# CEA-LIST/runia_core

Hardware: AMD Instinct MI355X
Metric: OOD scores/sec, LaREM 16-MC PCA-256 (ResNet-18 layer4 latent 512x4x4) (higher is better)
Workload: dtype f64

## Files before the change

### runia_core_amd/csrc/entropy_core.hpp

```cpp
#pragma once
#include "common.hpp"

namespace runia_entropy {

constexpr double kInf = __builtin_inf();

inline double digamma_diff(int n, int k) {
  double s = 0.0;
  for (int j = n - 1; j >= k; --j) s += 1.0 / (double)j;
  return s;
}

__device__ __forceinline__ void cswap(float& a, float& b) {
  float lo, hi;
  asm("v_min_f32 %0, %1, %2" : "=v"(lo) : "v"(a), "v"(b));
  asm("v_max_f32 %0, %1, %2" : "=v"(hi) : "v"(a), "v"(b));
  a = lo;
  b = hi;
}
__device__ __forceinline__ void cswap(double& a, double& b) {
  double lo, hi;
  asm("v_min_f64 %0, %1, %2" : "=v"(lo) : "v"(a), "v"(b));
  asm("v_max_f64 %0, %1, %2" : "=v"(hi) : "v"(a), "v"(b));
  a = lo;
  b = hi;
}

__device__ __forceinline__ void sort3(float& a, float& b, float& c) {
  float lo, md, hi;
  asm("v_min3_f32 %0, %1, %2, %3" : "=v"(lo) : "v"(a), "v"(b), "v"(c));
  asm("v_med3_f32 %0, %1, %2, %3" : "=v"(md) : "v"(a), "v"(b), "v"(c));
  asm("v_max3_f32 %0, %1, %2, %3" : "=v"(hi) : "v"(a), "v"(b), "v"(c));
  a = lo;
  b = md;
  c = hi;
}
__device__ __forceinline__ void sort3(double& a, double& b, double& c) {
  cswap(a, b);
  cswap(b, c);
  cswap(a, b);
}

template <int OFF, int NP, typename T>
__device__ __forceinline__ void sort16_at(T (&v)[NP]) {
#define RUNIA_S3(a, b, c) sort3(v[OFF + a], v[OFF + b], v[OFF + c]);
  RUNIA_S3(6, 7, 15) RUNIA_S3(10, 12, 13) RUNIA_S3(0, 2, 3) RUNIA_S3(1, 4, 5) RUNIA_S3(9, 11, 14)
  RUNIA_S3(3, 5, 15) RUNIA_S3(8, 13, 14) RUNIA_S3(2, 4, 7) RUNIA_S3(8, 10, 11) RUNIA_S3(9, 10, 12)
  RUNIA_S3(5, 7, 14) RUNIA_S3(0, 1, 6) RUNIA_S3(11, 12, 13) RUNIA_S3(3, 4, 6) RUNIA_S3(1, 2, 3)
  RUNIA_S3(5, 6, 13) RUNIA_S3(0, 8, 9) RUNIA_S3(1, 8, 9) RUNIA_S3(3, 7, 11) RUNIA_S3(13, 14, 15)
  RUNIA_S3(11, 12, 13) RUNIA_S3(4, 8, 11) RUNIA_S3(5, 7, 9) RUNIA_S3(2, 6, 10) RUNIA_S3(6, 7, 8)
  RUNIA_S3(3, 5, 6) RUNIA_S3(2, 3, 4) RUNIA_S3(9, 10, 11)
#undef RUNIA_S3
}

template <int OFF, int NP, typename T>
__device__ __forceinline__ void merge16x2_at(T (&v)[NP]) {
#define RUNIA_S3(a, b, c) sort3(v[OFF + a], v[OFF + b], v[OFF + c]);
#define RUNIA_S2(a, b) cswap(v[OFF + a], v[OFF + b]);
  RUNIA_S2(10, 26) RUNIA_S3(14, 26, 30) RUNIA_S3(12, 26, 28) RUNIA_S3(4, 12, 20) RUNIA_S3(0, 4, 16)
  RUNIA_S3(1, 4, 17) RUNIA_S3(3, 17, 19) RUNIA_S3(2, 10, 18) RUNIA_S3(15, 30, 31) RUNIA_S3(6, 10, 22)
  RUNIA_S3(5, 17, 21) RUNIA_S3(2, 3, 4) RUNIA_S3(13, 21, 29) RUNIA_S3(7, 19, 23) RUNIA_S3(11, 19, 27)
  RUNIA_S3(9, 21, 25) RUNIA_S3(7, 9, 17) RUNIA_S3(8, 20, 24) RUNIA_S3(15, 23, 27) RUNIA_S3(6, 7, 16)
  RUNIA_S3(11, 13, 17) RUNIA_S3(14, 18, 22) RUNIA_S3(8, 12, 16) RUNIA_S3(15, 19, 21) RUNIA_S3(9, 10, 12)
  RUNIA_S2(5, 6) RUNIA_S3(21, 22, 24) RUNIA_S3(18, 19, 20) RUNIA_S3(23, 25, 26) RUNIA_S3(15, 17, 18)
  RUNIA_S3(27, 28, 29) RUNIA_S3(14, 15, 16) RUNIA_S2(23, 24) RUNIA_S2(13, 14) RUNIA_S2(11, 12)
#undef RUNIA_S2
#undef RUNIA_S3
}

template <int NP, typename T>
__device__ __forceinline__ void sort_asc(T (&v)[NP]) {
  static_assert((NP & (NP - 1)) == 0, "power of two");
  if constexpr (NP == 8) {
#define RUNIA_S3(a, b, c) sort3(v[a], v[b], v[c]);
    RUNIA_S3(0, 5, 6) RUNIA_S3(1, 2, 3) RUNIA_S3(4, 6, 7) RUNIA_S3(0, 1, 4) RUNIA_S3(2, 5, 6) RUNIA_S3(3, 6, 7) RUNIA_S3(3, 4, 5) RUNIA_S3(1, 2, 3)
#undef RUNIA_S3
  } else {
    if constexpr (NP >= 16) {
      sort16_at<0>(v);
      if constexpr (NP >= 32) sort16_at<16>(v);
      if constexpr (NP >= 64) { sort16_at<32>(v); sort16_at<48>(v); }
      static_assert(NP <= 64, "add the 16-blocks of a larger sort here");
    }
    if constexpr (NP >= 32) {
      merge16x2_at<0>(v);
      if constexpr (NP >= 64) merge16x2_at<32>(v);
    }
#pragma unroll
    for (int p = (NP >= 32 ? 32 : (NP >= 16 ? 16 : 1)); p < NP; p <<= 1) {
#pragma unroll
      for (int k = p; k >= 1; k >>= 1) {
#pragma unroll
        for (int j = k % p; j + k < NP; j += 2 * k) {
#pragma unroll
          for (int i = 0; i < k; ++i) {
            if (i + j + k < NP && (i + j) / (2 * p) == (i + j + k) / (2 * p)) cswap(v[i + j], v[i + j + k]);
          }
        }
      }
    }
  }
}

__device__ __forceinline__ double fma_scalar_addend(double a, double b, double c) {
  double r;
  asm("v_fma_f64 %0, %1, %2, %3" : "=v"(r) : "v"(a), "v"(b), "s"(c));
  return r;
}

__device__ __forceinline__ double log_mantissa(double x, int& e_out) {
  int e;
  double f = frexp(x, &e);
  const bool low = f < 0.70710678118654752440;
  f = low ? f + f : f;
  e_out = low ? e - 1 : e;
  const double num = f - 1.0, den = f + 1.0;
  double r = __builtin_amdgcn_rcp(den);
  r = fma(fma(-den, r, 1.0), r, r);
  r = fma(fma(-den, r, 1.0), r, r);
  double q = num * r;
  q = fma(fma(-den, q, num), r, q);
  const double t = q * q;
  double p = 1.0 / 21.0;
  p = fma_scalar_addend(p, t, 1.0 / 19.0);
  p = fma_scalar_addend(p, t, 1.0 / 17.0);
  p = fma_scalar_addend(p, t, 1.0 / 15.0);
  p = fma_scalar_addend(p, t, 1.0 / 13.0);
  p = fma_scalar_addend(p, t, 1.0 / 11.0);
  p = fma_scalar_addend(p, t, 1.0 / 9.0);
  p = fma_scalar_addend(p, t, 1.0 / 7.0);
  p = fma_scalar_addend(p, t, 1.0 / 5.0);
  p = fma_scalar_addend(p, t, 1.0 / 3.0);
  const double q2 = q + q;
  return fma(q2 * t, p, q2);
}

template <int NP, int K, bool FULL = false>
__device__ __forceinline__ double column_log_sum(const float (&vs)[NP], int n, double min_dist) {
  double v[NP];
#pragma unroll
  for (int i = 0; i < NP; ++i) v[i] = (double)vs[i];
  double gap[NP][K];
#pragma unroll
  for (int a = 0; a < NP; ++a)
#pragma unroll
    for (int m = 1; m <= K; ++m) gap[a][m - 1] = (a + m < NP) ? v[a + m] - v[a] : kInf;
  double mant = 1.0;
  int esum = 0;
#pragma unroll
  for (int i0 = 0; i0 < NP; i0 += 4) {
    double prod = 1.0;
#pragma unroll
    for (int i = i0; i < i0 + 4 && i < NP; ++i) {
      double e = kInf;
      bool first = true;
#pragma unroll
      for (int j = 0; j <= K; ++j) {
        const int li = i - j, ri = i + (K - j);
        if (li < 0 || ri >= NP) continue;
        double cand;
        if (j == 0) cand = gap[i][K - 1];
        else if (j == K) cand = gap[li][K - 1];
        else cand = fmax(gap[li][j - 1], gap[i][K - j - 1]);
        e = first ? cand : fmin(e, cand);
        first = false;
      }
      e = fmax(e, min_dist);
      if (FULL || i < n) prod *= e;
    }
    int ex;
    const double m = frexp(prod, &ex);
    mant *= m;
    esum += ex;
  }
  int em;
  const double lf = log_mantissa(mant, em);
  return fma((double)(esum + em + (FULL ? NP : n)), 0.69314718055994530942, lf);
}

}
```

### runia_core_amd/csrc/mc_sampler.hip

```cpp
#include <type_traits>

#include "common.hpp"
#include "entropy_core.hpp"
#include "philox.hpp"
#include "div_consts.hpp"
#include "roi_source.hpp"

namespace {

using namespace runia_entropy;

constexpr int kMaxMC = 64;
typedef float f2 __attribute__((ext_vector_type(2)));
typedef float f4 __attribute__((ext_vector_type(4)));

#ifndef K0_NT_STORE
#define K0_NT_STORE 0
#endif
#ifndef K1_NT_STORE
#define K1_NT_STORE 0
#endif
template <int NT, typename T>
__device__ __forceinline__ void store_out(T* p, T v) {
  if constexpr (NT != 0) __builtin_nontemporal_store(v, p);
  else *p = v;
}

__device__ __forceinline__ void layer_consts(int cnt, int& m, float& flag, float& zh, float& zl) {
  const int a = cnt ? __ffs(cnt) - 1 : 0;
  m = cnt >> a;
  flag = __uint_as_float((unsigned)(127 - a) << 23);
  zh = cnt ? __uint_as_float(runia_div::kDivHi[(m - 1) >> 1]) : NAN;
  zl = cnt ? __uint_as_float(runia_div::kDivLo[(m - 1) >> 1]) : 0.f;
}

__device__ __forceinline__ float add_f32(float a, float b) {
  float r;
  asm("v_add_f32 %0, %1, %2" : "=v"(r) : "v"(a), "v"(b));
  return r;
}

__device__ __forceinline__ float div_newton(float u, float den, float r) {
  const float q = u * r;
  const float e = fmaf(-den, q, u);
  return fmaf(e, r, q);
}

template <int HT, int WT>
__host__ __device__ constexpr int mask_slot(int p) {
  if constexpr (HT % 2 == 0) {
    const int y = p / WT, xw = p - y * WT;
    return ((y >> 1) * WT + xw) * 2 + (y & 1);
  } else {
    return p;
  }
}

template <int HT, int WT>
__host__ __device__ constexpr int slot_position(int slot) {
  if constexpr (HT % 2 == 0) {
    const int e = slot & 1, t = slot >> 1;
    const int k = t / WT, xw = t - k * WT;
    return (2 * k + e) * WT + xw;
  } else {
    return slot;
  }
}

template <int HT, int WT>
__device__ __forceinline__ unsigned long long columns_below(int k) {
  unsigned long long row = (k >= 64) ? ~0ull : ((1ull << k) - 1ull), m = 0ull;
#pragma unroll
  for (int y = 0; y < HT; ++y) m |= row << (y * WT);
  return m;
}

constexpr int kMaskBitsWaves = 4;

template <int HT, int WT, int NP, bool REDRAW = false>
__global__ __launch_bounds__(64 * kMaskBitsWaves) void mc_mask_bits_kernel(const float* __restrict__ rnd,
                                                                           int64_t rand_stride,
                                                                           float* __restrict__ table, int64_t N,
                                                                           int n_mc, float gamma, int block_size,
                                                                           int identity, int sort_layers,
                                                                           uint64_t rng_seed, int64_t first_image) {
  constexpr int HW = HT * WT;
  static_assert(HW <= 64 && NP <= 64, "one drop layer per 64-bit word");
  constexpr bool DIV = (64 % HW == 0);
  constexpr int WORDS = (NP * HW + 63) / 64;
  constexpr unsigned long long FULL = (HW == 64) ? ~0ull : ((1ull << HW) - 1ull);
  const int lane = threadIdx.x & 63;
  const int64_t img = (int64_t)blockIdx.x * kMaskBitsWaves + (threadIdx.x >> 6);
  if (img >= N) return;
  const int bit0 = lane * HW, word0 = bit0 >> 6, off = bit0 & 63;
  const int pad = block_size / 2;

  auto seeds_of = [&](unsigned attempt) -> unsigned long long {
    float d[WORDS];
    if (rnd) {
      const float* r = rnd + img * rand_stride;
#pragma unroll
      for (int t = 0; t < WORDS; ++t) {
        const int i = lane + 64 * t;
        d[t] = (i < n_mc * HW) ? r[i] : 1.0f;
      }
    } else {
#pragma unroll
      for (int q = 0; q < (WORDS + 3) / 4; ++q) {
        const runia_philox::u4 b = runia_philox::lane_block(rng_seed, (uint64_t)(first_image + img), lane, q, attempt);
#pragma unroll
        for (int j = 0; j < 4; ++j) {
          const int t = 4 * q + j;
          if (t < WORDS) d[t] = (lane + 64 * t < n_mc * HW) ? runia_philox::component(b, j) : 1.0f;
        }
      }
    }
    unsigned long long lo = 0ull, hi = 0ull;
#pragma unroll
    for (int t = 0; t < WORDS; ++t) {
      const unsigned long long w = __ballot(d[t] < gamma);
      if (t == word0) lo = w;
      if (!DIV && t == word0 + 1) hi = w;
    }
    unsigned long long sd = lo >> off;
    if (!DIV && off + HW > 64) sd |= hi << (64 - off);
    return sd & FULL;
  };
  auto keep_of = [&](unsigned long long seed) -> unsigned long long {
    unsigned long long hx = 0ull;
    for (int dx = 0; dx < block_size; ++dx) {
      const int ox = dx - pad;
      if (ox >= WT || -ox >= WT) continue;
      hx |= (ox >= 0) ? ((seed >> ox) & columns_below<HT, WT>(WT - ox))
                      : ((seed << -ox) & ~columns_below<HT, WT>(-ox) & FULL);
    }
    unsigned long long dropped = 0ull;
    for (int dy = 0; dy < block_size; ++dy) {
      const int oy = dy - pad;
      if (oy >= HT || -oy >= HT) continue;
      dropped |= (oy >= 0) ? (hx >> (oy * WT)) : ((hx << (-oy * WT)) & FULL);
    }
    return ~dropped & FULL;
  };

  unsigned long long keep = identity ? FULL : keep_of(seeds_of(0u));
  if (REDRAW && !identity && !rnd) {
    for (unsigned attempt = 1; attempt <= 16u; ++attempt) {
      if (__ballot(lane < n_mc && keep == 0ull) == 0ull) break;
      const unsigned long long again = keep_of(seeds_of(attempt));
      if (keep == 0ull) keep = again;
    }
  }
  const int cnt = __popcll(keep);
  int m;
  float flag, zh, zl;
  layer_consts(cnt, m, flag, zh, zl);
  const int key = m ? m : 127;
  int rank = 0;
#pragma unroll
  for (int j = 0; j < NP; ++j) {
    const int o = __shfl(key, j, 64);
    rank += (j < n_mc) && ((o < key) || (o == key && j < lane));
  }
  if (!sort_layers) rank = lane;
  if (lane >= n_mc) return;
  float* out = table + img * (int64_t)(n_mc * (HW + 2));
  float* rec = out + rank * HW;
  if constexpr (HW % 4 == 0) {
#pragma unroll
    for (int c = 0; c < HW / 4; ++c) {
      f4 v;
      v.x = ((keep >> slot_position<HT, WT>(4 * c)) & 1ull) ? flag : 0.f;
      v.y = ((keep >> slot_position<HT, WT>(4 * c + 1)) & 1ull) ? flag : 0.f;
      v.z = ((keep >> slot_position<HT, WT>(4 * c + 2)) & 1ull) ? flag : 0.f;
      v.w = ((keep >> slot_position<HT, WT>(4 * c + 3)) & 1ull) ? flag : 0.f;
      store_out<K0_NT_STORE>(reinterpret_cast<f4*>(rec) + c, v);
    }
  } else {
#pragma unroll
    for (int q = 0; q < HW; ++q)
      store_out<K0_NT_STORE>(rec + q, ((keep >> slot_position<HT, WT>(q)) & 1ull) ? flag : 0.f);
  }
  store_out<K0_NT_STORE>(out + n_mc * HW + rank, zh);
  store_out<K0_NT_STORE>(out + n_mc * (HW + 1) + rank, zl);
}

constexpr int kLutRecDwords = 20, kLutSortDword = 18, kLutOddDword = 19;
constexpr int kLutLayerShift = 23, kLutClassShift = 27;
constexpr unsigned kLutOffsetMask = (1u << kLutLayerShift) - 1u;
constexpr size_t kLutKeys = 65536;
static_assert((kLutKeys - 1) * kLutRecDwords * 4 <= kLutOffsetMask, "a record's byte offset fits below the layer index");
constexpr size_t kLutRecords = (kLutOffsetMask + 1) / (kLutRecDwords * 4) + 2;
static_assert(kLutRecords * kLutRecDwords * 4 >= kLutOffsetMask + 1 + kLutRecDwords * 4, "every masked offset reads inside the table");

void flag_lut_fill_4x4(uint32_t* out, int block_size) {
  constexpr int HT = 4, WT = 4, HW = 16;
  const int pad = block_size / 2;
  for (size_t i = kLutKeys * kLutRecDwords; i < kLutRecords * kLutRecDwords; ++i) out[i] = 0u;
  for (unsigned key = 0; key < kLutKeys; ++key) {
    unsigned keep = 0;
    for (int y = 0; y < HT; ++y)
      for (int xw = 0; xw < WT; ++xw) {
        bool dropped = false;
        for (int yy = 0; yy < HT; ++yy)
          for (int xx = 0; xx < WT; ++xx)
            if (((key >> (yy * WT + xx)) & 1u) && yy - y >= -pad && yy - y < block_size - pad && xx - xw >= -pad &&
                xx - xw < block_size - pad)
              dropped = true;
        if (!dropped) keep |= 1u << (y * WT + xw);
      }
    const int cnt = __builtin_popcount(keep);
    const int a = cnt ? __builtin_ctz((unsigned)cnt) : 0;
    const int m = cnt >> a;
    const uint32_t flag = (uint32_t)(127 - a) << 23;
    uint32_t* rec = out + (size_t)key * kLutRecDwords;
    for (int slot = 0; slot < HW; ++slot) rec[slot] = ((keep >> slot_position<HT, WT>(slot)) & 1u) ? flag : 0u;
    rec[HW] = cnt ? runia_div::kDivHiC[(m - 1) >> 1] : 0x7fc00000u;
    rec[HW + 1] = cnt ? runia_div::kDivLoC[(m - 1) >> 1] : 0u;
    const unsigned cls = cnt ? (unsigned)(m - 1) >> 1 : 8u;
    rec[kLutSortDword] = (cls << kLutClassShift) | (key * (unsigned)(kLutRecDwords * 4));
    rec[kLutOddDword] = (uint32_t)m;
  }
}

__device__ __forceinline__ void sort16_uniform(unsigned (&v)[16]) {
#pragma unroll
  for (int p = 1; p < 16; p <<= 1) {
#pragma unroll
    for (int k = p; k >= 1; k >>= 1) {
#pragma unroll
      for (int j = k % p; j + k < 16; j += 2 * k) {
#pragma unroll
        for (int i = 0; i < k; ++i) {
          if (i + j + k < 16 && (i + j) / (2 * p) == (i + j + k) / (2 * p)) {
            const unsigned lo = v[i + j] < v[i + j + k] ? v[i + j] : v[i + j + k];
            const unsigned hi = v[i + j] < v[i + j + k] ? v[i + j + k] : v[i + j];
            v[i + j] = lo;
            v[i + j + k] = hi;
          }
        }
      }
    }
  }
}

#ifndef K1_BLOCK
#define K1_BLOCK 128
#endif
constexpr int kK1Block = K1_BLOCK;


template <int HT, int WT, int G>
__device__ __forceinline__ void roi_load_map(float (&u)[HT * WT], const RoiSource* __restrict__ src, int64_t roi, int c) {
  typedef const __attribute__((address_space(4))) unsigned* cptr;
  cptr tab = (cptr)(src->table + roi * (int64_t)src->roi_dwords);
  const unsigned image = tab[0];
  const __amdgpu_buffer_rsrc_t rsrc = __builtin_amdgcn_make_buffer_rsrc(
      const_cast<float*>(src->nhwc) + (int64_t)image * (src->image_bytes / 4), 0, (int)src->image_bytes, 0x00020000);
  const int voff = c * 4;
  cptr rows = tab + 8, cols = tab + 8 + 4 * (HT * G);
  constexpr float count = (float)(G * G);
  constexpr int SX = WT * G, SY = HT * G;
  unsigned ox_lo[SX], ox_hi[SX];
  float hx[SX], lx[SX];
#pragma unroll
  for (int sx = 0; sx < SX; ++sx) {
    ox_lo[sx] = cols[4 * sx];
    ox_hi[sx] = cols[4 * sx + 1];
    hx[sx] = __uint_as_float(cols[4 * sx + 2]);
    lx[sx] = __uint_as_float(cols[4 * sx + 3]);
  }
  float acc[HT * WT];
#pragma unroll
  for (int p = 0; p < HT * WT; ++p) acc[p] = 0.f;
  float tl[SX][2], th[SX][2];
  unsigned cur_lo = 0xffffffffu, cur_hi = 0xffffffffu;
#pragma unroll
  for (int sy = 0; sy < SY; ++sy) {
    const unsigned oy_lo = rows[4 * sy], oy_hi = rows[4 * sy + 1];
    const float hy = __uint_as_float(rows[4 * sy + 2]), ly = __uint_as_float(rows[4 * sy + 3]);
    if (oy_lo != cur_lo || oy_hi != cur_hi) {
      if (oy_lo == cur_hi) {
#pragma unroll
        for (int sx = 0; sx < SX; ++sx) { tl[sx][0] = th[sx][0]; tl[sx][1] = th[sx][1]; }
      } else {
#pragma unroll
        for (int sx = 0; sx < SX; ++sx) {
          tl[sx][0] = __builtin_bit_cast(float, __builtin_amdgcn_raw_buffer_load_b32(rsrc, voff, (int)(oy_lo + ox_lo[sx]), 0));
          tl[sx][1] = __builtin_bit_cast(float, __builtin_amdgcn_raw_buffer_load_b32(rsrc, voff, (int)(oy_lo + ox_hi[sx]), 0));
        }
      }
#pragma unroll
      for (int sx = 0; sx < SX; ++sx) {
        th[sx][0] = __builtin_bit_cast(float, __builtin_amdgcn_raw_buffer_load_b32(rsrc, voff, (int)(oy_hi + ox_lo[sx]), 0));
        th[sx][1] = __builtin_bit_cast(float, __builtin_amdgcn_raw_buffer_load_b32(rsrc, voff, (int)(oy_hi + ox_hi[sx]), 0));
      }
      cur_lo = oy_lo;
      cur_hi = oy_hi;
    }
    __builtin_amdgcn_sched_barrier(0);
#pragma unroll
    for (int sx = 0; sx < SX; ++sx) {
      const float w1 = hy * hx[sx], w2 = hy * lx[sx], w3 = ly * hx[sx], w4 = ly * lx[sx];
      const float val = w1 * tl[sx][0] + w2 * tl[sx][1] + w3 * th[sx][0] + w4 * th[sx][1];
      float& bin = acc[(sy / G) * WT + (sx / G)];
      bin += val;
      asm volatile("" : "+v"(bin));
    }
  }
#pragma unroll
  for (int p = 0; p < HT * WT; ++p) u[p] = acc[p] / count;
}

#ifndef K1_IMGS
#define K1_IMGS 1
#endif
template <int HT, int WT, int NP, int K, bool FULL, bool ENTROPY, int ROI_G, bool ZOUT, bool LUT = false>
__device__ __forceinline__ void mc_entropy_item(const float* __restrict__ x, const float* __restrict__ table,
                                                double* __restrict__ h, float* __restrict__ z_out,
                                                double* __restrict__ zero_fill, int64_t N, int C, int n_mc_rt,
                                                double min_dist, double const_term, double inv_n, int64_t img, int c,
                                                const float* __restrict__ rnd = nullptr, int64_t rand_stride = 0,
                                                float gamma = 0.f) {
  constexpr int HW = HT * WT;
  constexpr bool PAIRS = (HT % 2 == 0);
  const int n_mc = FULL ? NP : n_mc_rt;
  if (img >= N) return;
  unsigned long long seedw[LUT ? NP * HW / 64 : 1];
  if constexpr (LUT) {
    static_assert(!LUT || (HW == 16 && NP == 16 && FULL && !ZOUT && ROI_G == 0), "the geometry table is for 4x4 x 16 layers");
    const float* r = rnd + img * rand_stride + (threadIdx.x & 63);
#pragma unroll
    for (int t = 0; t < NP * HW / 64; ++t) seedw[t] = __ballot(r[64 * t] < gamma);
  }
  if (zero_fill && c == 0) zero_fill[img] = 0.0;
  if (c >= C) return;
  typedef const __attribute__((address_space(4))) unsigned* lut_ptr;
  const lut_ptr lut = (lut_ptr) reinterpret_cast<const unsigned*>(table);
  unsigned sv[LUT ? NP : 1];
  if constexpr (LUT) {
#pragma unroll
    for (int s = 0; s < NP; ++s) {
      const unsigned key = (unsigned)(seedw[s >> 2] >> (16 * (s & 3))) & 0xffffu;
      sv[s] = lut[key * kLutRecDwords + kLutSortDword] | ((unsigned)s << kLutLayerShift);
    }
    sort16_uniform(sv);
  }
  const float* mk = table + img * (int64_t)(n_mc * (HW + 2));
  const float* zhs = mk + n_mc * HW;
  const float* zls = zhs + n_mc;
  float u[HW];
  if constexpr (ROI_G > 0) {
    roi_load_map<HT, WT, ROI_G>(u, reinterpret_cast<const RoiSource*>(x), img, c);
  } else {
    const float* xc = x + (img * C + c) * (int64_t)HW;
    if constexpr (HW % 4 == 0) {
#pragma unroll
      for (int p = 0; p < HW / 4; ++p) {
        const float4 v = reinterpret_cast<const float4*>(xc)[p];
        u[4 * p] = v.x; u[4 * p + 1] = v.y; u[4 * p + 2] = v.z; u[4 * p + 3] = v.w;
      }
    } else {
#pragma unroll
      for (int p = 0; p < HW; ++p) u[p] = xc[p];
    }
  }
  constexpr bool w_pow2 = (WT & (WT - 1)) == 0, h_pow2 = (HT & (HT - 1)) == 0;
  constexpr bool hw_pow2 = w_pow2 && h_pow2;
  if constexpr (!hw_pow2) {
#pragma unroll
    for (int p = 0; p < HW; ++p) u[p] *= (float)HW;
  }
  const float rW = 1.0f / (float)WT, rH = 1.0f / (float)HT;
  float z[NP];
  float q[PAIRS ? 1 : HW];
  f2 q2[PAIRS ? HW / 2 : 1];
  unsigned cur_zh_bits = __float_as_uint(1.0f);
#pragma unroll
  for (int p = 0; p < HW; ++p) {
    if constexpr (PAIRS) q2[mask_slot<HT, WT>(p) >> 1][mask_slot<HT, WT>(p) & 1] = u[p];
    else q[p] = u[p];
  }
#ifndef K1_GCAP
#define K1_GCAP 128
#endif
  constexpr int GCAP = FULL ? K1_GCAP : K1_GCAP / 2;
  constexpr int G = (GCAP / HW < 1) ? 1 : ((GCAP / HW > NP) ? NP : GCAP / HW);
  if constexpr (!(FULL && NP % G == 0)) {
#pragma unroll
    for (int s = 0; s < NP; ++s) z[s] = INFINITY;
  }
#ifndef K1_TRIP_UNROLL
#define K1_TRIP_UNROLL 1
#endif
#pragma unroll K1_TRIP_UNROLL
  for (int s0 = 0; s0 < NP; s0 += G) {
    float znew[G];
    float dg[G], rg[G], mg[G][HW];
    const float* mk_t = mk + (FULL ? s0 * HW : 0);
    const float* zhs_t = zhs + (FULL ? s0 : 0);
    const float* zls_t = zls + (FULL ? s0 : 0);
#pragma unroll
    for (int g = 0; g < G; ++g) {
      if constexpr (LUT) {
        const lut_ptr rec = lut + (sv[g] & kLutOffsetMask) / 4u;
        dg[g] = __uint_as_float(rec[HW]);
        rg[g] = __uint_as_float(rec[HW + 1]);
#pragma unroll
        for (int p = 0; p < HW; ++p) mg[g][p] = __uint_as_float(rec[p]);
      } else {
        const int sc = FULL ? g : ((s0 + g < n_mc) ? s0 + g : n_mc - 1);
        dg[g] = zhs_t[sc];
        rg[g] = zls_t[sc];
#pragma unroll
        for (int p = 0; p < HW; ++p) mg[g][p] = mk_t[sc * HW + p];
      }
    }
#pragma unroll
    for (int g = 0; g < G; ++g) {
      const int s = s0 + g;
      znew[g] = INFINITY;
      if (FULL || s < n_mc) {
        const float zh = dg[g], zl = rg[g];
        if (__float_as_uint(zh) != cur_zh_bits) {
#pragma unroll
          for (int p = 0; p < HW; ++p) {
            const float qv = fmaf(u[p], zh, u[p] * zl);
            if constexpr (PAIRS) q2[mask_slot<HT, WT>(p) >> 1][mask_slot<HT, WT>(p) & 1] = qv;
            else q[p] = qv;
          }
          cur_zh_bits = __float_as_uint(zh);
        }
        const float* m = mg[g];
        float col;
        if constexpr (PAIRS) {
          float rows[HT];
#pragma unroll
          for (int k2 = 0; k2 < HT / 2; ++k2) {
            const f2* qq = q2 + k2 * WT;
            const float* mm = m + 2 * k2 * WT;
            f2 acc = qq[0] * (f2){mm[0], mm[1]};
#pragma unroll
            for (int xi = 1; xi < WT; ++xi) {
              const int xw = torch_chain<WT>(xi);
              acc = __builtin_elementwise_fma(qq[xw], (f2){mm[2 * xw], mm[2 * xw + 1]}, acc);
            }
            if constexpr (hw_pow2) {
            } else if constexpr (w_pow2) {
              acc = acc * (f2){rW, rW};
            } else {
              acc = (f2){div_newton(acc.x, (float)WT, rW), div_newton(acc.y, (float)WT, rW)};
            }
            rows[2 * k2] = acc.x;
            rows[2 * k2 + 1] = acc.y;
          }
          col = rows[0];
#pragma unroll
          for (int yi = 1; yi < HT; ++yi) col = add_f32(col, rows[torch_chain<HT>(yi)]);
        } else {
          float rm[HT];
#pragma unroll
          for (int y = 0; y < HT; ++y) {
            float rowsum = q[y * WT] * m[y * WT];
#pragma unroll
            for (int xi = 1; xi < WT; ++xi) {
              const int xw = torch_chain<WT>(xi);
              rowsum = fmaf(q[y * WT + xw], m[y * WT + xw], rowsum);
            }
            rm[y] = w_pow2 ? rowsum * rW : div_newton(rowsum, (float)WT, rW);
          }
          col = rm[0];
#pragma unroll
          for (int yi = 1; yi < HT; ++yi) col += rm[torch_chain<HT>(yi)];
        }
        if constexpr (hw_pow2 && PAIRS) znew[g] = col;
        else znew[g] = h_pow2 ? col * rH : div_newton(col, (float)HT, rH);
        if constexpr (ZOUT) {
          if (z_out) z_out[(img * n_mc + s) * (int64_t)C + c] = znew[g];
        }
      }
    }
#pragma unroll
    for (int i = NP - 1; i >= G; --i) z[i] = z[i - G];
#pragma unroll
    for (int g = 0; g < G; ++g) z[g] = znew[g];
    if constexpr (LUT) {
#pragma unroll
      for (int g = 0; g + G < NP; ++g) sv[g] = sv[g + G];
    }
  }
  if constexpr (ENTROPY) {
    float nan_probe = z[0];
#pragma unroll
    for (int s = 1; s < NP; ++s) nan_probe += z[s];
    const bool bad = nan_probe != nan_probe;
    sort_asc<NP>(z);
    double res = const_term + inv_n * column_log_sum<NP, K, FULL>(z, n_mc, min_dist);
    if (bad) res = NAN;
    store_out<K1_NT_STORE>(h + (img * C + c), res);
  }
}

template <int HT, int WT, int NP, int K, bool FULL, bool ENTROPY, int ROI_G, bool ZOUT>
#ifdef K1_WAVES
__attribute__((amdgpu_waves_per_eu(K1_WAVES, 8)))
#endif
__global__ __launch_bounds__(kK1Block) void mc_entropy_kernel(const float* __restrict__ x,
                                                          const float* __restrict__ table,
                                                          double* __restrict__ h, float* __restrict__ z_out,
                                                          double* __restrict__ zero_fill, int64_t N, int C,
                                                          int n_mc_rt, double min_dist, double const_term,
                                                          double inv_n) {
  const unsigned chunks = (unsigned)(C + kK1Block - 1) / kK1Block;
  const unsigned slot = blockIdx.x >> 3;
  const int c = (int)(slot % chunks) * kK1Block + threadIdx.x;
#pragma unroll 1
  for (int rep = 0; rep < K1_IMGS; ++rep) {
    const int64_t img = ((int64_t)(slot / chunks) * K1_IMGS + rep) * 8 + (blockIdx.x & 7);
    mc_entropy_item<HT, WT, NP, K, FULL, ENTROPY, ROI_G, ZOUT>(x, table, h, z_out, zero_fill, N, C, n_mc_rt, min_dist,
                                                              const_term, inv_n, img, c);
  }
}

template <int HT, int WT, int NP, int K>
__attribute__((amdgpu_waves_per_eu(6, 8)))
__global__ __launch_bounds__(kK1Block) void mc_entropy_lut_kernel(const float* __restrict__ x,
                                                              const float* __restrict__ rnd, int64_t rand_stride,
                                                              const float* __restrict__ lut, float gamma,
                                                              double* __restrict__ h, double* __restrict__ zero_fill,
                                                              int64_t N, int C, double min_dist, double const_term,
                                                              double inv_n) {
  const unsigned chunks = (unsigned)(C + kK1Block - 1) / kK1Block;
  const unsigned slot = blockIdx.x >> 3;
  const int c = (int)(slot % chunks) * kK1Block + threadIdx.x;
#pragma unroll 1
  for (int rep = 0; rep < K1_IMGS; ++rep) {
    const int64_t img = ((int64_t)(slot / chunks) * K1_IMGS + rep) * 8 + (blockIdx.x & 7);
    mc_entropy_item<HT, WT, NP, K, true, true, 0, false, true>(x, lut, h, nullptr, zero_fill, N, C, NP, min_dist, const_term,
                                                               inv_n, img, c, rnd, rand_stride, gamma);
  }
}

template <int HT, int WT, int NP, int K, bool FULL, int ROI_G>
void launch_mc_entropy(unsigned grid, hipStream_t s, const float* x, const float* table, double* h, float* z_out,
                       double* zero_fill, int64_t N, int C, int n_mc, double min_dist, double ct, double inv_n) {
  auto go = [&](auto kernel) {
    if constexpr (ROI_G == 0)
      RUNIA_LAUNCH_TIMED(kernel, grid, kK1Block, 0, s, x, table, h, z_out, zero_fill, N, C, n_mc, min_dist, ct, inv_n);
    else
      hipLaunchKernelGGL(kernel, dim3(grid), dim3(kK1Block), 0, s, x, table, h, z_out, zero_fill, N, C, n_mc, min_dist, ct,
                         inv_n);
  };
  if constexpr (HT == 4 && WT == 4) {
    if (!z_out) return go(mc_entropy_kernel<HT, WT, NP, K, FULL, true, ROI_G, false>);
  }
  go(mc_entropy_kernel<HT, WT, NP, K, FULL, true, ROI_G, true>);
}

template <int HH, int WW, int NPP>
void launch_mask(const float* rnd, int64_t rand_image_stride, float* table, int64_t N, int n_mc, float gamma,
                 int block_size, int identity, int sort_layers, uint64_t seed, int64_t first_image, int redraw,
                 hipStream_t s) {
  static_assert(HH * WW <= 64, "mc_mask_bits_kernel holds a drop layer in one 64-bit word");
  const unsigned grid = (unsigned)((N + kMaskBitsWaves - 1) / kMaskBitsWaves);
  if (redraw)
    mc_mask_bits_kernel<HH, WW, NPP, true><<<grid, 64 * kMaskBitsWaves, 0, s>>>(rnd, rand_image_stride, table, N, n_mc, gamma,
                                                                              block_size, identity, sort_layers, seed, first_image);
  else
    mc_mask_bits_kernel<HH, WW, NPP, false><<<grid, 64 * kMaskBitsWaves, 0, s>>>(rnd, rand_image_stride, table, N, n_mc, gamma,
                                                                               block_size, identity, sort_layers, seed, first_image);
}

__global__ void mc_draws_kernel(float* __restrict__ out, int64_t N, int per_image, uint64_t seed, int64_t first_image) {
  const int64_t i = (int64_t)blockIdx.x * blockDim.x + threadIdx.x;
  if (i >= N * per_image) return;
  const int64_t img = i / per_image;
  out[i] = runia_philox::draw(seed, (uint64_t)(first_image + img), (int)(i - img * per_image));
}
}

extern "C" size_t runia_mc_entropy_workspace_bytes(int64_t N, int H, int W, int n_mc) {
  if (N <= 0 || H <= 0 || W <= 0 || n_mc <= 0) return 0;
  return (size_t)N * (size_t)n_mc * (size_t)(H * W + 2) * sizeof(float);
}

static unsigned k1_grid(int64_t N, int C) {
  return (unsigned)((((N + 7) / 8 + K1_IMGS - 1) / K1_IMGS) * 8 * ((C + kK1Block - 1) / kK1Block));
}

#define RUNIA_MCE_SHAPES(F) \
  F(4, 4, 16, 5) F(4, 4, 32, 5) F(4, 4, 8, 5) F(2, 2, 16, 5) F(2, 2, 32, 5) F(7, 7, 16, 5) F(7, 7, 32, 5) F(8, 8, 16, 5) F(8, 8, 32, 5)

#define RUNIA_ROI_MCE_SHAPES(X)                                                                                    \
  X(7, 7, 16, 5, 2) X(7, 7, 32, 5, 2) X(7, 7, 16, 5, 1) X(7, 7, 32, 5, 1)                                          \
  X(4, 4, 16, 5, 2) X(4, 4, 32, 5, 2) X(8, 8, 16, 5, 2) X(8, 8, 32, 5, 2)

template <int V> using int_c = std::integral_constant<int, V>;

template <class F>
int mc_for_shape(int H, int W, int n_mc, int k, F&& f, bool any_k = false) {
#define RUNIA_MCE(HH, WW, NPP, KK)                                                                 \
  if (H == HH && W == WW && n_mc <= NPP && n_mc > NPP / 2 && (k == KK || any_k)) {                \
    if (n_mc == NPP) f(int_c<HH>{}, int_c<WW>{}, int_c<NPP>{}, int_c<KK>{}, std::true_type{});     \
    else f(int_c<HH>{}, int_c<WW>{}, int_c<NPP>{}, int_c<KK>{}, std::false_type{});                \
    return 1;                                                                                      \
  }
  RUNIA_MCE_SHAPES(RUNIA_MCE)
#undef RUNIA_MCE
  return 0;
}

template <class F>
int roi_mc_for_shape(int PH, int PW, int n_mc, int k, int sampling_ratio, F&& f) {
#define RUNIA_ROI_MCE(HH, WW, NPP, KK, GG)                                                                    \
  if (PH == HH && PW == WW && n_mc <= NPP && n_mc > NPP / 2 && k == KK && sampling_ratio == GG) {             \
    if (n_mc == NPP) f(int_c<HH>{}, int_c<WW>{}, int_c<NPP>{}, int_c<KK>{}, int_c<GG>{}, std::true_type{});   \
    else f(int_c<HH>{}, int_c<WW>{}, int_c<NPP>{}, int_c<KK>{}, int_c<GG>{}, std::false_type{});              \
    return 1;                                                                                                 \
  }
  RUNIA_ROI_MCE_SHAPES(RUNIA_ROI_MCE)
#undef RUNIA_ROI_MCE
  return 0;
}

extern "C" int runia_mc_entropy_supported(int H, int W, int n_mc, int k) {
  return k < n_mc && mc_for_shape(H, W, n_mc, k, [](auto...) {});
}

extern "C" int runia_roi_mc_entropy_supported(int PH, int PW, int n_mc, int k, int sampling_ratio) {
  return
      runia_mc_entropy_supported(PH, PW, n_mc, k) && roi_mc_for_shape(PH, PW, n_mc, k, sampling_ratio, [](auto...) {});
}

constexpr int64_t kMaxImages = 65535;
constexpr int kNoArg = 1;

static int mc_args_ok(int64_t N, int C, int H, int W, int n_mc, int block_size, int k, bool has_ws = false,
                      const void* ws = nullptr, size_t ws_bytes = 0) {
  if (N < 0 || N > kMaxImages || C <= 0 || H <= 0 || W <= 0 || n_mc < 2 || n_mc > kMaxMC || block_size < 1 || k < 1 || k >= n_mc)
    return RUNIA_E_INVALID;
  const bool refused = ws_refused(ws, ws_bytes, runia_mc_entropy_workspace_bytes(N, H, W, n_mc), 16);
  return (N > 0 && has_ws && refused) ? RUNIA_E_WORKSPACE : RUNIA_OK;
}

static bool k1_operands_ok(const float* x, const void* out, int H, int W, int n_mc, int k) {
  return x && out && runia_mc_entropy_supported(H, W, n_mc, k) && ((((uintptr_t)x) & 15) == 0 || (H * W) % 4 != 0);
}

static int mc_mask_table(const float* rnd, int64_t rand_image_stride, void* workspace, size_t workspace_bytes,
                         int64_t N, int H, int W, int n_mc, double drop_prob, int block_size, int sort_layers,
                         runia_stream_t stream, bool counter = false, uint64_t seed = 0, int64_t first_image = 0,
                         int redraw = 0) {
  if (int rc = mc_args_ok(N, kNoArg, H, W, n_mc, block_size, kNoArg, true, workspace, workspace_bytes)) return rc;
  if (N == 0) return RUNIA_OK;
  const int identity = (drop_prob == 0.0);
  if (!identity && !rnd && !counter) return RUNIA_E_INVALID;
  if (counter) rnd = nullptr;
  float* table = reinterpret_cast<float*>(workspace);
  const float gamma = (float)(drop_prob / (double)(block_size * block_size));
  hipStream_t s = as_stream(stream);
  if (!mc_for_shape(H, W, n_mc, 0, [&](auto hh, auto ww, auto np, auto, auto) {
        launch_mask<hh, ww, np>(rnd, rand_image_stride, table, N, n_mc, gamma, block_size, identity, sort_layers, seed,
                                first_image, redraw, s);
      }, true))
    return RUNIA_E_INVALID;
  return runia_check_launch();
}

extern "C" int runia_mc_mask_table_f32(const float* rnd, int64_t rand_image_stride, void* workspace,
                                       size_t workspace_bytes, int64_t N, int H, int W, int n_mc, double drop_prob,
                                       int block_size, runia_stream_t stream) {
  return mc_mask_table(rnd, rand_image_stride, workspace, workspace_bytes, N, H, W, n_mc, drop_prob, block_size, 1,
                       stream);
}

extern "C" int runia_mc_stack_table_f32(const float* x, const float* rnd, int64_t rand_image_stride, float* z,
                                        void* workspace, size_t workspace_bytes, int64_t N, int C, int H, int W,
                                        int n_mc, double drop_prob, int block_size, runia_stream_t stream) {
  if (int rc = mc_args_ok(N, C, H, W, n_mc, kNoArg, kNoArg, true, workspace, workspace_bytes)) return rc;
  if (N == 0) return RUNIA_OK;
  if (!k1_operands_ok(x, z, H, W, n_mc, 5)) return RUNIA_E_INVALID;
  if (int rc = mc_mask_table(rnd, rand_image_stride, workspace, workspace_bytes, N, H, W, n_mc, drop_prob,
                             block_size, 0, stream))
    return rc;
  const float* table = reinterpret_cast<const float*>(workspace);
  hipStream_t s = as_stream(stream);
  if (!mc_for_shape(H, W, n_mc, 5, [&](auto hh, auto ww, auto np, auto kk, auto full) {
        mc_entropy_kernel<hh, ww, np, kk, full, false, 0, true><<<k1_grid(N, C), kK1Block, 0, s>>>(
            x, table, nullptr, z, nullptr, N, C, n_mc, 0.0, 0.0, 0.0);
      }))
    return RUNIA_E_INVALID;
  return runia_check_launch();
}

extern "C" int runia_mc_entropy_from_table_f32(const float* x, const void* workspace, size_t workspace_bytes,
                                               double* h, float* z_out, double* zero_fill, int64_t N, int C,
                                               int H, int W, int n_mc, int k, double min_dist,
                                               runia_stream_t stream) {
  if (int rc = mc_args_ok(N, C, H, W, n_mc, kNoArg, k, true, workspace, workspace_bytes)) return rc;
  if (N == 0) return RUNIA_OK;
  if (!k1_operands_ok(x, h, H, W, n_mc, k)) return RUNIA_E_INVALID;
  const float* table = reinterpret_cast<const float*>(workspace);
  const double ct = digamma_diff(n_mc, k), inv_n = 1.0 / (double)n_mc;
  hipStream_t s = as_stream(stream);
  if (!mc_for_shape(H, W, n_mc, k, [&](auto hh, auto ww, auto np, auto kk, auto full) {
        launch_mc_entropy<hh, ww, np, kk, full, 0>(k1_grid(N, C), s, x, table, h, z_out, zero_fill, N, C, n_mc, min_dist, ct,
                                                   inv_n);
      }))
    return RUNIA_E_INVALID;
  return runia_check_launch();
}

extern "C" int runia_mc_entropy_f32(const float* x, const float* rnd, int64_t rand_image_stride, double* h,
                                    float* z_out, double* zero_fill, void* workspace, size_t workspace_bytes,
                                    int64_t N, int C, int H, int W, int n_mc, double drop_prob, int block_size,
                                    int k, double min_dist, runia_stream_t stream) {
  if (int rc = mc_args_ok(N, C, H, W, n_mc, block_size, k)) return rc;
  if (N == 0) return RUNIA_OK;
  if (!k1_operands_ok(x, h, H, W, n_mc, k)) return RUNIA_E_INVALID;
  if (drop_prob != 0.0 && !rnd) return RUNIA_E_INVALID;
  if (int rc = runia_mc_mask_table_f32(rnd, rand_image_stride, workspace, workspace_bytes, N, H, W, n_mc, drop_prob,
                                       block_size, stream))
    return rc;
  return runia_mc_entropy_from_table_f32(x, workspace, workspace_bytes, h, z_out, zero_fill, N, C, H, W, n_mc, k,
                                         min_dist, stream);
}

extern "C" size_t runia_mc_flag_lut_bytes(int H, int W, int block_size) {
  if (H != 4 || W != 4 || block_size < 1) return 0;
  return kLutRecords * kLutRecDwords * sizeof(uint32_t);
}

extern "C" int runia_mc_flag_lut_fill(void* host_out, size_t bytes, int H, int W, int block_size) {
  const size_t need = runia_mc_flag_lut_bytes(H, W, block_size);
  if (need == 0 || !host_out || (((uintptr_t)host_out) & 3) != 0) return RUNIA_E_INVALID;
  if (bytes < need) return RUNIA_E_WORKSPACE;
  flag_lut_fill_4x4(reinterpret_cast<uint32_t*>(host_out), block_size);
  return RUNIA_OK;
}

extern "C" int runia_mc_entropy_lut_supported(int H, int W, int n_mc, int k, int block_size) {
  return H == 4 && W == 4 && n_mc == 16 && k == 5 && block_size >= 1;
}

extern "C" int runia_mc_entropy_lut_f32(const float* x, const float* rnd, int64_t rand_image_stride, const void* lut,
                                        size_t lut_bytes, double* h, double* zero_fill, int64_t N, int C, int H, int W,
                                        int n_mc, double drop_prob, int block_size, int k, double min_dist,
                                        runia_stream_t stream) {
  if (rand_image_stride < 0 || !runia_mc_entropy_lut_supported(H, W, n_mc, k, block_size)) return RUNIA_E_INVALID;
  if (!(drop_prob > 0.0)) return RUNIA_E_INVALID;
  if (int rc = mc_args_ok(N, C, H, W, n_mc, block_size, k)) return rc;
  if (N == 0) return RUNIA_OK;
  if (!rnd || !k1_operands_ok(x, h, H, W, n_mc, k)) return RUNIA_E_INVALID;
  if (ws_refused(lut, lut_bytes, runia_mc_flag_lut_bytes(H, W, block_size), 4)) return RUNIA_E_WORKSPACE;
  const float gamma = (float)(drop_prob / (double)(block_size * block_size));
  const double ct = digamma_diff(n_mc, k), inv_n = 1.0 / (double)n_mc;
  RUNIA_LAUNCH_TIMED((mc_entropy_lut_kernel<4, 4, 16, 5>), k1_grid(N, C), kK1Block, 0, as_stream(stream), x, rnd,
                     rand_image_stride, reinterpret_cast<const float*>(lut), gamma, h, zero_fill, N, C, min_dist, ct, inv_n);
  return runia_check_launch();
}

struct RoiMcPlan { float* masks; size_t masks_bytes; char* tab; };
static RoiMcPlan roi_mc_plan(WsWalk& w, int64_t K, int PH, int PW, int n_mc, int sampling_ratio) {
  RoiMcPlan p;
  p.masks = w.take<float>(runia_mc_entropy_workspace_bytes(K, PH, PW, n_mc) / sizeof(float), 256);
  p.masks_bytes = w.used();
  p.tab = w.take<char>(runia_roi_sample_table_bytes(K, PH, PW, sampling_ratio));
  return p;
}
extern "C" size_t runia_roi_mc_entropy_workspace_bytes(int64_t K, int PH, int PW, int n_mc, int sampling_ratio) {
  if (K <= 0 || sampling_ratio < 1) return 0;
  return ws_bytes([&](WsWalk& w) { roi_mc_plan(w, K, PH, PW, n_mc, sampling_ratio); });
}
extern "C" int runia_roi_mc_entropy_f32(const float* feat_nhwc, const float* boxes, const int* batch_idx, const float* rnd,
                                        int64_t rand_image_stride, double* h, float* z_out, void* workspace,
                                        size_t workspace_bytes, int64_t K, int64_t B, int C, int H, int W, int PH, int PW,
                                        double spatial_scale, int sampling_ratio, int aligned, int n_mc, double drop_prob,
                                        int block_size, int k, double min_dist, runia_stream_t stream) {
  if (B <= 0) return RUNIA_E_INVALID;
  if (int rc = mc_args_ok(K, C, H, W, n_mc, block_size, k)) return rc;
  if (K == 0) return RUNIA_OK;
  if (!feat_nhwc || !boxes || !h || (B > 1 && !batch_idx)) return RUNIA_E_INVALID;
  if (!runia_roi_mc_entropy_supported(PH, PW, n_mc, k, sampling_ratio)) return RUNIA_E_INVALID;
  if ((int64_t)H * W * C * 4 >= ((int64_t)1 << 30)) return RUNIA_E_INVALID;
  if (drop_prob != 0.0 && !rnd) return RUNIA_E_INVALID;
  WsWalk w(workspace);
  const RoiMcPlan plan = roi_mc_plan(w, K, PH, PW, n_mc, sampling_ratio);
  if (ws_refused(workspace, workspace_bytes, w.used(), 16)) return RUNIA_E_WORKSPACE;
  const size_t masks = plan.masks_bytes;
  if (int rc = runia_mc_mask_table_f32(rnd, rand_image_stride, workspace, masks, K, PH, PW, n_mc, drop_prob, block_size, stream))
    return rc;
  char* tab = plan.tab;
  hipStream_t s = as_stream(stream);
  if (int rc = runia_roi_sample_table(feat_nhwc, boxes, batch_idx, tab, workspace_bytes - masks, K, B, C, H, W, PH, PW,
                                      spatial_scale, sampling_ratio, aligned, s))
    return rc;
  const float* table = plan.masks;
  const float* src = reinterpret_cast<const float*>(tab);
  const double ct = digamma_diff(n_mc, k), inv_n = 1.0 / (double)n_mc;
  if (!roi_mc_for_shape(PH, PW, n_mc, k, sampling_ratio, [&](auto hh, auto ww, auto np, auto kk, auto gg, auto full) {
        launch_mc_entropy<hh, ww, np, kk, full, gg>(k1_grid(K, C), s, src, table, h, z_out, nullptr, K, C, n_mc, min_dist, ct,
                                                    inv_n);
      }))
    return RUNIA_E_INVALID;
  return runia_check_launch();
}

extern "C" int runia_mc_draws_f32(float* out, int64_t N, int n_mc, int H, int W, uint64_t seed, int64_t first_image,
                                  runia_stream_t stream) {
  if (N < 0 || n_mc < 1 || H <= 0 || W <= 0 || first_image < 0 || (int64_t)n_mc * H * W > (1 << 20))
    return RUNIA_E_INVALID;
  if (N == 0) return RUNIA_OK;
  if (!out) return RUNIA_E_INVALID;
  const int64_t total = N * n_mc * H * W;
  if ((total + 255) / 256 > 0x7fffffffLL) return RUNIA_E_INVALID;
  mc_draws_kernel<<<(unsigned)((total + 255) / 256), 256, 0, as_stream(stream)>>>(out, N, n_mc * H * W, seed,
                                                                                first_image);
  return runia_check_launch();
}

extern "C" int runia_mc_mask_table_counter_f32(uint64_t seed, int64_t first_image, void* workspace,
                                               size_t workspace_bytes, int64_t N, int H, int W, int n_mc,
                                               double drop_prob, int block_size, int redraw_dead_layers,
                                               runia_stream_t stream) {
  if (first_image < 0) return RUNIA_E_INVALID;
  return mc_mask_table(nullptr, 0, workspace, workspace_bytes, N, H, W, n_mc, drop_prob, block_size, 1, stream, true,
                       seed, first_image, redraw_dead_layers ? 1 : 0);
}

extern "C" int runia_mc_entropy_counter_f32(const float* x, uint64_t seed, int64_t first_image, double* h,
                                            float* z_out, double* zero_fill, void* workspace, size_t workspace_bytes,
                                            int64_t N, int C, int H, int W, int n_mc, double drop_prob,
                                            int block_size, int k, double min_dist, int redraw_dead_layers,
                                            runia_stream_t stream) {
  if (first_image < 0) return RUNIA_E_INVALID;
  if (int rc = mc_args_ok(N, C, H, W, n_mc, block_size, k)) return rc;
  if (N == 0) return RUNIA_OK;
  if (!k1_operands_ok(x, h, H, W, n_mc, k)) return RUNIA_E_INVALID;
  if (int rc = runia_mc_mask_table_counter_f32(seed, first_image, workspace, workspace_bytes, N, H, W, n_mc,
                                               drop_prob, block_size, redraw_dead_layers, stream))
    return rc;
  return runia_mc_entropy_from_table_f32(x, workspace, workspace_bytes, h, z_out, zero_fill, N, C, H, W, n_mc, k,
                                         min_dist, stream);
}
```

Measured before the change: 65.36 million.

## Slide gap computation in LUT entropy path and raise LUT kernel wave target

For the LUT entropy kernel, the column log-sum now converts sorted values to double and computes the k-nearest gaps in a sliding fashion inside the main loop instead of materialising all values and gaps up front. Empty asm barriers pin the order of these steps, and the min-distance clamp uses an SGPR operand, so fewer double registers stay live at once. The LUT kernel's waves_per_eu minimum rises from 6 to 8 to exploit the lower register pressure for higher occupancy. The risk is spills or a worse instruction schedule if the compiler cannot fit the forced occupancy.

```diff
diff --git a/runia_core_amd/csrc/entropy_core.hpp b/runia_core_amd/csrc/entropy_core.hpp
--- a/runia_core_amd/csrc/entropy_core.hpp
+++ b/runia_core_amd/csrc/entropy_core.hpp
@@ -105,6 +105,12 @@
 __device__ __forceinline__ double fma_scalar_addend(double a, double b, double c) {
   double r;
   asm("v_fma_f64 %0, %1, %2, %3" : "=v"(r) : "v"(a), "v"(b), "s"(c));
+  return r;
+}
+
+__device__ __forceinline__ double max_scalar(double a, double c) {
+  double r;
+  asm("v_max_f64 %0, %1, %2" : "=v"(r) : "v"(a), "s"(c));
   return r;
 }
 
@@ -135,16 +141,22 @@
   return fma(q2 * t, p, q2);
 }
 
-template <int NP, int K, bool FULL = false>
+template <int NP, int K, bool FULL = false, bool SLIDE = false>
 __device__ __forceinline__ double column_log_sum(const float (&vs)[NP], int n, double min_dist) {
+  static_assert(!SLIDE || (FULL && NP > K), "the sliding form is for full columns");
   double v[NP];
-#pragma unroll
-  for (int i = 0; i < NP; ++i) v[i] = (double)vs[i];
   double gap[NP][K];
-#pragma unroll
-  for (int a = 0; a < NP; ++a)
-#pragma unroll
-    for (int m = 1; m <= K; ++m) gap[a][m - 1] = (a + m < NP) ? v[a + m] - v[a] : kInf;
+  if constexpr (SLIDE) {
+#pragma unroll
+    for (int i = 0; i < K; ++i) v[i] = (double)vs[i];
+  } else {
+#pragma unroll
+    for (int i = 0; i < NP; ++i) v[i] = (double)vs[i];
+#pragma unroll
+    for (int a = 0; a < NP; ++a)
+#pragma unroll
+      for (int m = 1; m <= K; ++m) gap[a][m - 1] = (a + m < NP) ? v[a + m] - v[a] : kInf;
+  }
   double mant = 1.0;
   int esum = 0;
 #pragma unroll
@@ -152,6 +164,15 @@
     double prod = 1.0;
 #pragma unroll
     for (int i = i0; i < i0 + 4 && i < NP; ++i) {
+      if constexpr (SLIDE) {
+        if (i + K < NP) {
+          v[i + K] = (double)vs[i + K];
+          asm volatile("" : "+v"(v[i + K]));
+        }
+#pragma unroll
+        for (int m = 1; m <= K; ++m)
+          if (i + m < NP) gap[i][m - 1] = v[i + m] - v[i];
+      }
       double e = kInf;
       bool first = true;
 #pragma unroll
@@ -165,8 +186,10 @@
         e = first ? cand : fmin(e, cand);
         first = false;
       }
-      e = fmax(e, min_dist);
+      if constexpr (SLIDE) e = max_scalar(e, min_dist);
+      else e = fmax(e, min_dist);
       if (FULL || i < n) prod *= e;
+      if constexpr (SLIDE) asm volatile("" : "+v"(prod));
     }
     int ex;
     const double m = frexp(prod, &ex);
diff --git a/runia_core_amd/csrc/mc_sampler.hip b/runia_core_amd/csrc/mc_sampler.hip
--- a/runia_core_amd/csrc/mc_sampler.hip
+++ b/runia_core_amd/csrc/mc_sampler.hip
@@ -248,6 +248,10 @@
 #define K1_BLOCK 128
 #endif
 constexpr int kK1Block = K1_BLOCK;
+#ifndef K1_LUT_WAVES
+#define K1_LUT_WAVES 8
+#endif
+static_assert(K1_LUT_WAVES >= 1 && K1_LUT_WAVES <= 8, "at most eight waves per SIMD");
 
 
 template <int HT, int WT, int G>
@@ -495,9 +499,11 @@
     for (int s = 1; s < NP; ++s) nan_probe += z[s];
     const bool bad = nan_probe != nan_probe;
     sort_asc<NP>(z);
-    double res = const_term + inv_n * column_log_sum<NP, K, FULL>(z, n_mc, min_dist);
+    double res = const_term + inv_n * column_log_sum<NP, K, FULL, LUT>(z, n_mc, min_dist);
     if (bad) res = NAN;
-    store_out<K1_NT_STORE>(h + (img * C + c), res);
+    int c_out = c;
+    if constexpr (LUT) asm volatile("" : "+v"(c_out));
+    store_out<K1_NT_STORE>(h + (img * C + c_out), res);
   }
 }
 
@@ -523,7 +529,7 @@
 }
 
 template <int HT, int WT, int NP, int K>
-__attribute__((amdgpu_waves_per_eu(6, 8)))
+__attribute__((amdgpu_waves_per_eu(K1_LUT_WAVES, 8)))
 __global__ __launch_bounds__(kK1Block) void mc_entropy_lut_kernel(const float* __restrict__ x,
                                                               const float* __restrict__ rnd, int64_t rand_stride,
                                                               const float* __restrict__ lut, float gamma,
```

Result: no change. 66.06 million (median of 6 runs) (+1.1%).
